# ibm-granite/dolomite-engine

Measured on NVIDIA H100. Metric: tokens_per_sec, higher is better.
Workload: dtype bf16

## Files before the change

dolomite_engine_b200/csrc/attention_fwd.cu:

```cuda
#include "attention_common.cuh"
#include "../../include/dolomite_b200.h"

using namespace dolo;

namespace {

constexpr int FWD_THREADS = 256;
constexpr int KV_STAGES = 2;

struct FwdParams {
    __nv_bfloat16* out;
    float* lse;
    const int32_t* cu_seqlens;
    int n_docs;
    int64_t T;
    int n_groups, q_per_group;
    int n_heads;
    float scale_log2;
    float scale;
    AttnDropout drop;
    int head_chunk;
    int n_tile_slots;
};

template <int HD>
__global__ void __launch_bounds__(FWD_THREADS, 1)
    attn_fwd_kernel(const __grid_constant__ CUtensorMap tmap64, const __grid_constant__ CUtensorMap tmapR,
                    const FwdParams p) {
    using CH = HeadChunks<HD>;
    constexpr int TILE_BYTES = CH::tile_bytes(ATT_TILE);

    int ti, head;
    attn_cta_order(p.head_chunk, p.n_tile_slots, ti, head);
    ti = p.n_tile_slots - 1 - ti;
    const TileLoc loc = locate_tile(p.cu_seqlens, p.n_docs, ti);
    if (!loc.valid) return;
    const int group = head / p.q_per_group, slot = head % p.q_per_group;
    const int q_col = (group * (p.q_per_group + 2) + slot) * HD;
    const int k_col = (group * (p.q_per_group + 2) + p.q_per_group) * HD;
    const int v_col = k_col + HD;
    const int q0 = loc.tile * ATT_TILE;
    const int n_kv = loc.tile + 1;

    extern __shared__ uint8_t smem_raw[];
    uint8_t* smem = smem_align_1024(smem_raw);
    uint8_t* sQ = smem;
    uint8_t* sK = sQ + TILE_BYTES;
    uint8_t* sV = sK + KV_STAGES * TILE_BYTES;
    uint64_t* bars = reinterpret_cast<uint64_t*>(sV + KV_STAGES * TILE_BYTES);
    uint64_t* q_full = bars;
    uint64_t* kv_full = bars + 1;
    uint64_t* kv_empty = bars + 3;

    const int wg = threadIdx.x >> 7, warp = threadIdx.x >> 5, lane = threadIdx.x & 31;

    auto load_kv = [&](int j, int s) {
        mbar_expect_tx(&kv_full[s], 2 * TILE_BYTES);
        tma_load_chunked<HD, ATT_TILE>(sK + s * TILE_BYTES, &tmap64, &tmapR, &kv_full[s], k_col, loc.doc_start + j * ATT_TILE);
        tma_load_chunked<HD, ATT_TILE>(sV + s * TILE_BYTES, &tmap64, &tmapR, &kv_full[s], v_col, loc.doc_start + j * ATT_TILE);
    };
    if (threadIdx.x == 0) {
        if (CH::NC64 > 0) tma_prefetch_desc(&tmap64);
        if (CH::REM > 0) tma_prefetch_desc(&tmapR);
        mbar_init(q_full, 1);
        for (int i = 0; i < KV_STAGES; ++i) {
            mbar_init(&kv_full[i], 1);
            mbar_init(&kv_empty[i], FWD_THREADS / 32);
        }
        mbar_fence_init();
        mbar_expect_tx(q_full, TILE_BYTES);
        tma_load_chunked<HD, ATT_TILE>(sQ, &tmap64, &tmapR, q_full, q_col, loc.doc_start + q0);
        for (int j = 0; j < KV_STAGES && j < n_kv; ++j) load_kv(j, j);
    }
    __syncthreads();

    const int wr = (warp & 3) * 16 + (lane >> 2);
    const int wc = 2 * (lane & 3);
    const int qr[2] = {q0 + wg * 64 + wr, q0 + wg * 64 + wr + 8};
    const bool drop = p.drop.threshold != 0;
    const uint32_t head_key = dropout_head_key(uint32_t(head), p.drop.key0, p.drop.key1);
    const uint32_t sq = smem_u32(sQ);

    float o[HD / 2];
#pragma unroll
    for (int i = 0; i < HD / 2; ++i) o[i] = 0.f;
    float m_run[2] = {-INFINITY, -INFINITY}, l_run[2] = {0.f, 0.f};

    mbar_wait(q_full, 0, 10);
    for (int j = 0; j < n_kv; ++j) {
        const int s = j & (KV_STAGES - 1);
        mbar_wait(&kv_full[s], (j / KV_STAGES) & 1, 11);
        const uint32_t sk = smem_u32(sK + s * TILE_BYTES), sv = smem_u32(sV + s * TILE_BYTES);
        float sc[ATT_TILE / 2];
        wgmma_fence();
#pragma unroll
        for (int c = 0; c < CH::NCHUNK; ++c) {
            const int w = CH::width(c);
#pragma unroll
            for (int k = 0; k < w / 16; ++k)
                wgmma_ss<ATT_TILE, 0, 0>(sc, chunk_desc_kmajor(sq + CH::offset(c, ATT_TILE) + wg * 64 * 2 * w, w, k),
                                         chunk_desc_kmajor(sk + CH::offset(c, ATT_TILE), w, k), (c != 0 || k != 0) ? 1u : 0u);
        }
        wgmma_commit();
        wgmma_wait<0>();
        reg_fence<ATT_TILE / 2>(sc);

        const bool diag = j == loc.tile;
        const int kbase = j * ATT_TILE + wc;
#pragma unroll
        for (int h = 0; h < 2; ++h) {
            float mx = m_run[h];
#pragma unroll
            for (int b = 0; b < ATT_TILE / 8; ++b)
#pragma unroll
                for (int e = 0; e < 2; ++e) {
                    float& x = sc[4 * b + 2 * h + e];
                    if (diag && kbase + 8 * b + e > qr[h]) x = -INFINITY;
                    mx = fmaxf(mx, x);
                }
            mx = fmaxf(mx, __shfl_xor_sync(0xffffffffu, mx, 1));
            mx = fmaxf(mx, __shfl_xor_sync(0xffffffffu, mx, 2));
            const float corr = fast_exp2((m_run[h] - mx) * p.scale_log2);
            const float neg_m = -mx * p.scale_log2;
            float lsum = 0.f;
#pragma unroll
            for (int b = 0; b < ATT_TILE / 8; ++b)
#pragma unroll
                for (int e = 0; e < 2; ++e) {
                    float& x = sc[4 * b + 2 * h + e];
                    float pr = fast_exp2(fmaf(x, p.scale_log2, neg_m));
                    lsum += pr;
                    if (drop)
                        pr *= attn_drop_scale(p.drop, head_key, loc.doc_start + qr[h], loc.doc_start + kbase + 8 * b + e);
                    x = pr;
                }
            l_run[h] = l_run[h] * corr + lsum;
            m_run[h] = mx;
#pragma unroll
            for (int b = 0; b < HD / 8; ++b) {
                o[4 * b + 2 * h] *= corr;
                o[4 * b + 2 * h + 1] *= corr;
            }
        }
        uint32_t pa[ATT_TILE / 16][4];
#pragma unroll
        for (int kk = 0; kk < ATT_TILE / 16; ++kk) acc_to_a_frag(sc, kk, pa[kk]);

        wgmma_fence();
#pragma unroll
        for (int c = 0; c < CH::NCHUNK; ++c) {
#pragma unroll
            for (int kk = 0; kk < ATT_TILE / 16; ++kk) {
                if (CH::width(c) == 64)
                    wgmma_rs<64, 1>(o + CH::col(c) / 2, pa[kk], chunk_desc_mnmajor(sv + CH::offset(c, ATT_TILE), 64, kk), 1u);
                else
                    wgmma_rs<(CH::REM ? CH::REM : 16), 1>(o + CH::col(c) / 2, pa[kk],
                                                          chunk_desc_mnmajor(sv + CH::offset(c, ATT_TILE), CH::REM, kk), 1u);
            }
        }
        wgmma_commit();
        wgmma_wait<0>();
        reg_fence<HD / 2>(o);
        if (lane == 0) mbar_arrive(&kv_empty[s]);
        if (threadIdx.x == 0 && j + KV_STAGES < n_kv) {
            mbar_wait(&kv_empty[s], (j / KV_STAGES) & 1, 12);
            load_kv(j + KV_STAGES, s);
        }
        __syncwarp();
    }

#pragma unroll
    for (int h = 0; h < 2; ++h) {
        float l = l_run[h];
        l += __shfl_xor_sync(0xffffffffu, l, 1);
        l += __shfl_xor_sync(0xffffffffu, l, 2);
        if (qr[h] >= loc.doc_len) continue;
        const float inv_l = l > 0.f ? 1.f / l : 0.f;
        const int64_t row = loc.doc_start + qr[h];
        __nv_bfloat16* orow = p.out + row * (int64_t(p.n_heads) * HD) + int64_t(head) * HD + wc;
#pragma unroll
        for (int b = 0; b < HD / 8; ++b)
            *reinterpret_cast<uint32_t*>(orow + 8 * b) = pack_bf16(o[4 * b + 2 * h] * inv_l, o[4 * b + 2 * h + 1] * inv_l);
        if ((lane & 3) == 0) p.lse[int64_t(head) * p.T + row] = m_run[h] * p.scale + logf(l);
    }
}

template <int HD>
int launch_fwd(const void* qkv, int64_t row_stride, const FwdParams& p, cudaStream_t st) {
    using CH = HeadChunks<HD>;
    CUtensorMap t64, tR;
    int rc = attn_make_maps<HD>(qkv, row_stride, p.T, &t64, &tR);
    if (rc) return rc;
    constexpr int smem_bytes = 1024 + (1 + 2 * KV_STAGES) * CH::tile_bytes(ATT_TILE) + 128;
    static_assert(smem_bytes <= 232448, "attention forward shared memory budget exceeded");
    auto kern = attn_fwd_kernel<HD>;
    static bool attr_set = false;
    if (!attr_set) {
        DOLO_CUDA_OK(cudaFuncSetAttribute(kern, cudaFuncAttributeMaxDynamicSharedMemorySize, smem_bytes));
        attr_set = true;
    }
    const int64_t max_tiles = (p.T + ATT_TILE - 1) / ATT_TILE + p.n_docs;
    DOLO_REQUIRE(max_tiles == p.n_tile_slots && max_tiles * p.n_heads < (1ll << 31), "attn_fwd: grid too large");
    dim3 grid((unsigned)(max_tiles * p.n_heads));
    kern<<<grid, FWD_THREADS, smem_bytes, st>>>(t64, tR, p);
    DOLO_LAUNCH_OK("attn_varlen_fwd");
    return DOLO_OK;
}

}

uint32_t dolo_dropout_threshold(float p);

extern "C" int dolomite_b200_attn_varlen_fwd(const void* qkv, int64_t row_stride, void* out, float* lse,
                                             const int32_t* cu_seqlens, int n_docs, int64_t T, int max_seqlen,
                                             int n_groups, int q_per_group, int head_dim, float softmax_scale,
                                             void* stream) {
    return dolomite_b200_attn_varlen_fwd_dropout(qkv, row_stride, out, lse, cu_seqlens, n_docs, T, max_seqlen, n_groups,
                                                 q_per_group, head_dim, softmax_scale, 0.f, 0, 0, stream);
}

extern "C" int dolomite_b200_attn_varlen_fwd_dropout(const void* qkv, int64_t row_stride, void* out, float* lse,
                                                     const int32_t* cu_seqlens, int n_docs, int64_t T, int max_seqlen,
                                                     int n_groups, int q_per_group, int head_dim, float softmax_scale,
                                                     float dropout_p, uint32_t key0, uint32_t key1, void* stream) {
    DOLO_REQUIRE(dropout_p >= 0.f && dropout_p < 1.f, "attn_fwd: dropout_p=%f must be in [0, 1)", double(dropout_p));
    DOLO_REQUIRE(n_docs >= 0 && T >= 0, "attn_fwd: negative sizes");
// ... 36 lines not shown
```

dolomite_engine_b200/csrc/common.cuh:

```cuda
#pragma once

#include <cuda.h>
#include <cuda_bf16.h>
#include <cuda_runtime.h>
#include <stdint.h>
#include <stdio.h>

extern "C" const char* dolomite_b200_last_error();
int dolo_set_error(const char* fmt, ...);
int dolo_check_cuda(cudaError_t e, const char* what);

#define DOLO_CUDA_OK(expr)                                             \
    do {                                                               \
        cudaError_t _e = (expr);                                       \
        if (_e != cudaSuccess) return dolo_check_cuda(_e, #expr);      \
    } while (0)

#define DOLO_REQUIRE(cond, ...)                                        \
    do {                                                               \
        if (!(cond)) return dolo_set_error(__VA_ARGS__);               \
    } while (0)

#define DOLO_LAUNCH_OK(name)                                           \
    do {                                                               \
// ... 52 lines not shown
    uint32_t ok;
    asm volatile(
        "{\n\t"
        ".reg .pred p;\n\t"
        "mbarrier.try_wait.parity.shared::cta.b64 p, [%1], %2;\n\t"
        "selp.u32 %0, 1, 0, p;\n\t"
        "}\n"
        : "=r"(ok)
        : "r"(smem_u32(bar)), "r"(parity)
        : "memory");
    return ok != 0;
}

#ifndef DOLO_WATCHDOG_CYCLES
#define DOLO_WATCHDOG_CYCLES (8000000000LL)
#endif
__device__ __forceinline__ void mbar_wait(uint64_t* bar, uint32_t parity, int tag = 0) {
    (void)tag;
    if (mbar_try_wait(bar, parity)) return;
    long long t0 = clock64();
    while (!mbar_try_wait(bar, parity)) {
        if (clock64() - t0 > DOLO_WATCHDOG_CYCLES) __trap();
    }
}

__device__ __forceinline__ void fence_proxy_async_smem() {
    asm volatile("fence.proxy.async.shared::cta;" ::: "memory");
}

__device__ __forceinline__ void named_bar_sync(uint32_t id, uint32_t nthreads) {
    asm volatile("bar.sync %0, %1;" ::"r"(id), "r"(nthreads) : "memory");
}

__device__ __forceinline__ void tma_prefetch_desc(const CUtensorMap* m) {
    asm volatile("prefetch.tensormap [%0];" ::"l"(reinterpret_cast<uint64_t>(m)) : "memory");
}
__device__ __forceinline__ void tma_load_2d(void* smem_dst, const CUtensorMap* m, uint64_t* bar, int c0, int c1) {
    asm volatile(
        "cp.async.bulk.tensor.2d.shared::cluster.global.mbarrier::complete_tx::bytes [%0], [%1, {%3, %4}], [%2];"
        ::"r"(smem_u32(smem_dst)), "l"(reinterpret_cast<uint64_t>(m)), "r"(smem_u32(bar)), "r"(c0), "r"(c1)
        : "memory");
}
constexpr uint64_t TMA_HINT_NORMAL = 0x1000000000000000ull;
constexpr uint64_t TMA_HINT_EVICT_FIRST = 0x12F0000000000000ull;
constexpr uint64_t TMA_HINT_EVICT_LAST = 0x14F0000000000000ull;
__device__ __forceinline__ void tma_load_2d_hint(void* smem_dst, const CUtensorMap* m, uint64_t* bar, int c0, int c1,
                                                 uint64_t hint) {
    asm volatile(
        "cp.async.bulk.tensor.2d.shared::cluster.global.mbarrier::complete_tx::bytes.L2::cache_hint [%0], [%1, {%3, %4}], [%2], %5;"
        ::"r"(smem_u32(smem_dst)), "l"(reinterpret_cast<uint64_t>(m)), "r"(smem_u32(bar)), "r"(c0), "r"(c1), "l"(hint)
        : "memory");
}
__device__ __forceinline__ void tma_load_3d(void* smem_dst, const CUtensorMap* m, uint64_t* bar, int c0, int c1,
                                            int c2) {
    asm volatile(
        "cp.async.bulk.tensor.3d.shared::cluster.global.mbarrier::complete_tx::bytes [%0], [%1, {%3, %4, %5}], [%2];"
        ::"r"(smem_u32(smem_dst)), "l"(reinterpret_cast<uint64_t>(m)), "r"(smem_u32(bar)), "r"(c0), "r"(c1), "r"(c2)
        : "memory");
}
__device__ __forceinline__ void tma_store_2d(const CUtensorMap* m, const void* smem_src, int c0, int c1) {
    asm volatile("cp.async.bulk.tensor.2d.global.shared::cta.bulk_group [%0, {%2, %3}], [%1];" ::"l"(
                     reinterpret_cast<uint64_t>(m)),
                 "r"(smem_u32(smem_src)), "r"(c0), "r"(c1)
                 : "memory");
}
__device__ __forceinline__ void tma_reduce_add_2d(const CUtensorMap* m, const void* smem_src, int c0, int c1) {
// ... 37 lines not shown
}
__device__ __forceinline__ void cluster_sync_all() {
    asm volatile("barrier.cluster.arrive.release.aligned;" ::: "memory");
    asm volatile("barrier.cluster.wait.acquire.aligned;" ::: "memory");
}

__device__ __forceinline__ uint64_t gmma_desc(uint32_t saddr, uint32_t lbo_bytes, uint32_t sbo_bytes, uint32_t layout_type) {
    uint64_t d = 0;
    d |= uint64_t((saddr & 0x3FFFFu) >> 4);
    d |= uint64_t((lbo_bytes >> 4) & 0x3FFFu) << 16;
    d |= uint64_t((sbo_bytes >> 4) & 0x3FFFu) << 32;
    d |= uint64_t(layout_type & 3u) << 62;
    return d;
}
__device__ __forceinline__ void wgmma_fence() { asm volatile("wgmma.fence.sync.aligned;" ::: "memory"); }
__device__ __forceinline__ void wgmma_commit() { asm volatile("wgmma.commit_group.sync.aligned;" ::: "memory"); }
template <int N>
__device__ __forceinline__ void wgmma_wait() {
    asm volatile("wgmma.wait_group.sync.aligned %0;" ::"n"(N) : "memory");
}
template <int N>
__device__ __forceinline__ void setmaxnreg_dec() {
    asm volatile("setmaxnreg.dec.sync.aligned.u32 %0;" ::"n"(N));
}
template <int N>
__device__ __forceinline__ void setmaxnreg_inc() {
    asm volatile("setmaxnreg.inc.sync.aligned.u32 %0;" ::"n"(N));
}
template <int N>
__device__ __forceinline__ void reg_fence(float* d) {
#pragma unroll
    for (int i = 0; i < N; ++i) asm volatile("" : "+f"(d[i])::"memory");
}


__device__ __forceinline__ uint32_t pack_bf16(float lo, float hi) {
    __nv_bfloat162 v = __floats2bfloat162_rn(lo, hi);
    return *reinterpret_cast<uint32_t*>(&v);
}
__device__ __forceinline__ float bf16_lo(uint32_t v) { return __uint_as_float(v << 16); }
__device__ __forceinline__ float bf16_hi(uint32_t v) { return __uint_as_float(v & 0xFFFF0000u); }
__device__ __forceinline__ float bf16_round(float x) { return __bfloat162float(__float2bfloat16_rn(x)); }
__device__ __forceinline__ void acc_to_a_frag(const float* d, int kk, uint32_t (&a)[4]) {
    a[0] = pack_bf16(d[8 * kk + 0], d[8 * kk + 1]);
    a[1] = pack_bf16(d[8 * kk + 2], d[8 * kk + 3]);
    a[2] = pack_bf16(d[8 * kk + 4], d[8 * kk + 5]);
    a[3] = pack_bf16(d[8 * kk + 6], d[8 * kk + 7]);
}

__device__ __forceinline__ uint32_t lowbias32(uint32_t x) {
    x ^= x >> 16;
    x *= 0x21f0aaadu;
    x ^= x >> 15;
    x *= 0x735a2d97u;
    x ^= x >> 15;
    return x;
}
__device__ __forceinline__ uint32_t dropout_hash_flat(uint64_t e, uint32_t key0, uint32_t key1) {
    return lowbias32(lowbias32(uint32_t(e) ^ key0) + uint32_t(e >> 32) + key1);
}
__device__ __forceinline__ uint32_t dropout_head_key(uint32_t head, uint32_t key0, uint32_t key1) {
    return lowbias32(head * 0xC2B2AE3Du + key0) ^ key1;
}
__device__ __forceinline__ uint32_t dropout_hash_qk(uint32_t q, uint32_t k, uint32_t head_key) {
    return lowbias32((q * 0x9E3779B1u) ^ (k * 0x85EBCA77u) ^ head_key);
}
// ... 21 lines not shown
```

dolomite_engine_b200/csrc/gemm.cu:

```cuda
#include <string.h>

#include "common.cuh"
#include "wgmma.cuh"
#include "../../include/dolomite_b200.h"

using namespace dolo;

namespace {

constexpr int BM = 128;
constexpr int BN = 128;
constexpr int BK = 64;
constexpr int STAGES = 6;
constexpr int A_STAGE_BYTES = BM * BK * 2;
constexpr int B_STAGE_BYTES = BN * BK * 2;
constexpr int STAGE_BYTES = A_STAGE_BYTES + B_STAGE_BYTES;
constexpr int GEMM_THREADS = 384;
constexpr int SMEM_BYTES = 1024  + STAGES * STAGE_BYTES + 256 ;
static_assert(SMEM_BYTES <= 232448, "shared memory budget exceeded (227 KB per block on sm_90)");

template <int TN>
struct Ring {
    static_assert(TN == 128 || TN == 256, "tile width 128 or 256");
    static constexpr int STAGES = TN == 256 ? 4 : 6;
    static constexpr int B_BYTES = TN * BK * 2;
    static constexpr int STAGE_BYTES = A_STAGE_BYTES + B_BYTES;
    static constexpr int SMEM_BYTES = 1024  + STAGES * STAGE_BYTES + 256 ;
    static_assert(SMEM_BYTES <= 232448, "shared memory budget exceeded (227 KB per block on sm_90)");
};

constexpr int PRODUCER_REGS = 40;
constexpr int CONSUMER_REGS = 232;
static_assert(PRODUCER_REGS * 128 + 2 * CONSUMER_REGS * 128 <= 65536, "register file exceeded");

constexpr double TILE256_COST = 1.81;

constexpr int MAXP = 4;

struct GemmMaps {
    CUtensorMap a[MAXP], b[MAXP];
};

struct Problem {
    void* D;
    const void* C;
    const __nv_bfloat16* bias;
    int64_t ldd, ldc;
    int M, N;
    int num_m, num_n, num_kb;
    int group_m;
    int tile_start;
    float alpha, beta;
    uint64_t hint_a, hint_b;
};

struct GemmParams {
    Problem pr[MAXP];
    int n_prob;
    int num_tiles;
    int d_is_f32;
    int grouped;
    const int* m_tile_group;
    const int* a_row_index;
    const void* gather_a;
    int64_t gather_lda;
    int gather_k;
    int b_group_rows;
    const int* group_k_offsets;
    int num_groups;
    int64_t d_group_stride;
};

struct TileInfo {
    int q;
    int m_blk, n_blk, grp, kb0, kb1;
    bool valid;
};

__device__ __forceinline__ void tile_coords(int t, int num_m, int num_n, int gm, int& m_blk, int& n_blk) {
    const int per_group = gm * num_n;
    const int group = t / per_group;
    const int first_m = group * gm;
    const int gsize = min(num_m - first_m, gm);
    const int r = t - group * per_group;
    m_blk = first_m + r % gsize;
    n_blk = r / gsize;
}

__device__ __forceinline__ TileInfo tile_info(int t, const GemmParams& p) {
    TileInfo ti;
    ti.q = 0;
#pragma unroll
    for (int i = 1; i < MAXP; ++i)
        if (i < p.n_prob && t >= p.pr[i].tile_start) ti.q = i;
    const Problem& pr = p.pr[ti.q];
    t -= pr.tile_start;
    ti.grp = 0;
    ti.kb0 = 0;
    ti.kb1 = pr.num_kb;
    ti.valid = true;
    if (p.grouped == 3) {
        const int per = pr.num_m * pr.num_n;
        const int split = t / per;
        tile_coords(t - split * per, pr.num_m, pr.num_n, pr.group_m, ti.m_blk, ti.n_blk);
        const int kb_per = (pr.num_kb + p.num_groups - 1) / p.num_groups;
        ti.kb0 = split * kb_per;
        ti.kb1 = min(pr.num_kb, ti.kb0 + kb_per);
        ti.valid = ti.kb1 > ti.kb0;
    } else if (p.grouped == 2) {
        const int per = pr.num_m * pr.num_n;
        ti.grp = t / per;
        tile_coords(t - ti.grp * per, pr.num_m, pr.num_n, pr.group_m, ti.m_blk, ti.n_blk);
        ti.kb0 = p.group_k_offsets[ti.grp] / BK;
        ti.kb1 = p.group_k_offsets[ti.grp + 1] / BK;
        ti.valid = ti.kb1 > ti.kb0;
    } else {
        tile_coords(t, pr.num_m, pr.num_n, pr.group_m, ti.m_blk, ti.n_blk);
        if (p.grouped == 1) {
            ti.grp = p.m_tile_group[ti.m_blk];
            ti.valid = ti.grp >= 0;
        }
    }
    return ti;
}

template <bool A_MN, bool B_MN, int TN>
__global__ void __launch_bounds__(GEMM_THREADS, 1)
    gemm_bf16_kernel(const __grid_constant__ GemmMaps maps, const __grid_constant__ GemmParams p) {
    constexpr int STAGES = Ring<TN>::STAGES;
    constexpr int B_STAGE_BYTES = Ring<TN>::B_BYTES;
    constexpr int STAGE_BYTES = Ring<TN>::STAGE_BYTES;
    extern __shared__ uint8_t smem_raw[];
    uint8_t* smem = smem_align_1024(smem_raw);
    uint8_t* smem_a = smem;
    uint8_t* smem_b = smem + STAGES * A_STAGE_BYTES;
    uint64_t* bars = reinterpret_cast<uint64_t*>(smem + STAGES * STAGE_BYTES);
    uint64_t* full_bar = bars;
    uint64_t* empty_bar = bars + STAGES;

    const int wg = threadIdx.x >> 7;
    const int warp = threadIdx.x >> 5;
    const int lane = threadIdx.x & 31;
    const int num_tiles = p.num_tiles;
    const bool gather = TN == 128 && !A_MN && p.a_row_index != nullptr;

    if (threadIdx.x == 0) {
        for (int q = 0; q < p.n_prob; ++q) {
            if (!gather) tma_prefetch_desc(&maps.a[q]);
            tma_prefetch_desc(&maps.b[q]);
        }
        for (int i = 0; i < STAGES; ++i) {
            mbar_init(&full_bar[i], gather ? 33 : 1);
            mbar_init(&empty_bar[i], 8);
        }
        mbar_fence_init();
    }
    __syncthreads();

    if (wg == 0) {
        if constexpr (TN == 256) setmaxnreg_dec<PRODUCER_REGS>();
        if (warp != 0) return;
        if (gather) {
            const __nv_bfloat16* A = static_cast<const __nv_bfloat16*>(p.gather_a);
            int stage = 0;
            uint32_t phase = 0;
            for (int t = blockIdx.x; t < num_tiles; t += gridDim.x) {
                const TileInfo ti = tile_info(t, p);
                if (!ti.valid) continue;
                const CUtensorMap* tmap_b = &maps.b[ti.q];
                const int b_outer = ti.grp * p.b_group_rows;
                const int4 src = *reinterpret_cast<const int4*>(p.a_row_index + int64_t(ti.m_blk) * BM + lane * 4);
                const int srow[4] = {src.x, src.y, src.z, src.w};
                for (int kb = ti.kb0; kb < ti.kb1; ++kb) {
                    mbar_wait(&empty_bar[stage], phase ^ 1, 1);
                    uint8_t* sa = smem_a + stage * A_STAGE_BYTES;
                    uint8_t* sb = smem_b + stage * B_STAGE_BYTES;
                    if (lane == 0) {
                        mbar_expect_tx(&full_bar[stage], B_STAGE_BYTES);
                        if (!B_MN) {
                            tma_load_2d(sb, tmap_b, &full_bar[stage], kb * BK, b_outer + ti.n_blk * BN);
                        } else {
#pragma unroll
                            for (int i = 0; i < BN / 64; ++i)
                                tma_load_2d(sb + i * (BK * 128), tmap_b, &full_bar[stage], ti.n_blk * BN + i * 64,
                                            b_outer + kb * BK);
                        }
                    }
// ... 23 lines not shown
                const CUtensorMap* tmap_b = &maps.b[ti.q];
                const uint64_t ha = p.pr[ti.q].hint_a, hb = p.pr[ti.q].hint_b;
                const int m_blk = ti.m_blk, n_blk = ti.n_blk;
                const int b_outer = (p.grouped == 1) ? ti.grp * p.b_group_rows : 0;
                for (int kb = ti.kb0; kb < ti.kb1; ++kb) {
                    mbar_wait(&empty_bar[stage], phase ^ 1, 1);
                    uint8_t* sa = smem_a + stage * A_STAGE_BYTES;
                    uint8_t* sb = smem_b + stage * B_STAGE_BYTES;
                    mbar_expect_tx(&full_bar[stage], STAGE_BYTES);
                    if (!A_MN) {
                        tma_load_2d_hint(sa, tmap_a, &full_bar[stage], kb * BK, m_blk * BM, ha);
                    } else {
#pragma unroll
                        for (int i = 0; i < BM / 64; ++i)
                            tma_load_2d_hint(sa + i * (BK * 128), tmap_a, &full_bar[stage], m_blk * BM + i * 64, kb * BK, ha);
                    }
                    if (!B_MN) {
                        tma_load_2d_hint(sb, tmap_b, &full_bar[stage], kb * BK, b_outer + n_blk * TN, hb);
                    } else {
#pragma unroll
                        for (int i = 0; i < TN / 64; ++i)
                            tma_load_2d_hint(sb + i * (BK * 128), tmap_b, &full_bar[stage], n_blk * TN + i * 64,
                                             b_outer + kb * BK, hb);
                    }
                    if (++stage == STAGES) { stage = 0; phase ^= 1; }
                }
            }
        }
        return;
    }

    if constexpr (TN == 256) setmaxnreg_inc<CONSUMER_REGS>();
    const int cw = wg - 1;
    const int wr = (warp & 3) * 16 + (lane >> 2);
    const int wc = 2 * (lane & 3);
    int stage = 0;
    uint32_t phase = 0;
    float acc[TN / 2];
    for (int t = blockIdx.x; t < num_tiles; t += gridDim.x) {
        const TileInfo ti = tile_info(t, p);
        const Problem& pr = p.pr[ti.q];
        const int64_t row0 = int64_t(ti.m_blk) * BM + cw * 64 + wr;
        const int col0 = ti.n_blk * TN + wc;
        if (!ti.valid) {
            if (p.grouped == 2 && p.d_is_f32 && pr.C == nullptr) {
                float* D = static_cast<float*>(pr.D) + int64_t(ti.grp) * p.d_group_stride;
#pragma unroll
                for (int h = 0; h < 2; ++h) {
                    const int64_t row = row0 + 8 * h;
                    if (row >= pr.M) continue;
                    for (int j = 0; j < TN / 8; ++j)
                        if (col0 + 8 * j < pr.N)
                            *reinterpret_cast<float2*>(D + row * pr.ldd + col0 + 8 * j) = make_float2(0.f, 0.f);
                }
            }
            continue;
        }
        int prev_stage = -1;
        for (int kb = ti.kb0; kb < ti.kb1; ++kb) {
            mbar_wait(&full_bar[stage], phase, 3);
            wgmma_fence();
            const uint32_t sa = smem_u32(smem_a + stage * A_STAGE_BYTES);
            const uint32_t sb = smem_u32(smem_b + stage * B_STAGE_BYTES);
#pragma unroll
            for (int k = 0; k < BK / 16; ++k) {
                const uint64_t adesc = A_MN ? gmma_desc(sa + cw * (BK * 128) + k * 2048, BK * 128, 1024, 1)
                                            : gmma_desc(sa + cw * (64 * 128) + k * 32, 16, 1024, 1);
                const uint64_t bdesc = B_MN ? gmma_desc(sb + k * 2048, BK * 128, 1024, 1) : gmma_desc(sb + k * 32, 16, 1024, 1);
                wgmma_ss<TN, A_MN ? 1 : 0, B_MN ? 1 : 0>(acc, adesc, bdesc, (kb != ti.kb0 || k != 0) ? 1u : 0u);
            }
            wgmma_commit();
            wgmma_wait<1>();
            if (prev_stage >= 0 && lane == 0) mbar_arrive(&empty_bar[prev_stage]);
            prev_stage = stage;
            if (++stage == STAGES) { stage = 0; phase ^= 1; }
        }
        wgmma_wait<0>();
        reg_fence<TN / 2>(acc);
        if (prev_stage >= 0 && lane == 0) mbar_arrive(&empty_bar[prev_stage]);

        const int64_t d_off = (p.grouped == 2) ? int64_t(ti.grp) * p.d_group_stride : 0;
        const float alpha = pr.alpha, beta = pr.beta;
        const __nv_bfloat16* bias = pr.bias;
        const int N = pr.N;
#pragma unroll
        for (int j = 0; j < TN / 8; ++j) {
            const int col = col0 + 8 * j;
            if (col >= N) continue;
            float b0 = 0.f, b1 = 0.f;
            if (bias != nullptr) {
                const uint32_t bv = *reinterpret_cast<const uint32_t*>(bias + col);
                b0 = bf16_lo(bv);
                b1 = bf16_hi(bv);
            }
#pragma unroll
            for (int h = 0; h < 2; ++h) {
                const int64_t row = row0 + 8 * h;
                if (row >= pr.M) continue;
                float v0 = (acc[4 * j + 2 * h] + b0) * alpha;
                float v1 = (acc[4 * j + 2 * h + 1] + b1) * alpha;
                if (p.d_is_f32) {
                    float* d = static_cast<float*>(pr.D) + d_off + row * pr.ldd + col;
                    if (p.grouped == 3) {
                        asm volatile("red.global.add.v2.f32 [%0], {%1, %2};" ::"l"(d), "f"(v0), "f"(v1) : "memory");
                        continue;
                    }
                    if (pr.C) {
                        const float2 c2 = *reinterpret_cast<const float2*>(static_cast<const float*>(pr.C) + d_off + row * pr.ldc + col);
                        v0 += beta * c2.x;
                        v1 += beta * c2.y;
                    }
                    *reinterpret_cast<float2*>(d) = make_float2(v0, v1);
                } else {
                    __nv_bfloat16* d = static_cast<__nv_bfloat16*>(pr.D) + d_off + row * pr.ldd + col;
                    if (pr.C) {
                        const uint32_t cv =
                            *reinterpret_cast<const uint32_t*>(static_cast<const __nv_bfloat16*>(pr.C) + d_off + row * pr.ldc + col);
                        v0 += beta * bf16_lo(cv);
                        v1 += beta * bf16_hi(cv);
                    }
                    *reinterpret_cast<uint32_t*>(d) = pack_bf16(v0, v1);
                }
            }
        }
    }
}

int gemm_workers() {
    const int sms = dolo_num_sms() - dolo_option_gemm_sm_margin();
    return sms < 1 ? 1 : sms;
}

template <bool A_MN, bool B_MN, int TN>
int launch_gemm(const GemmMaps& maps, const GemmParams& p, cudaStream_t st) {
    auto kern = gemm_bf16_kernel<A_MN, B_MN, TN>;
    constexpr int smem_bytes = Ring<TN>::SMEM_BYTES;
    static bool attr_set = false;
    if (!attr_set) {
        DOLO_CUDA_OK(cudaFuncSetAttribute(kern, cudaFuncAttributeMaxDynamicSharedMemorySize, smem_bytes));
        attr_set = true;
    }
    const int sms = gemm_workers();
    const int grid = p.num_tiles < sms ? p.num_tiles : sms;
    kern<<<grid, GEMM_THREADS, smem_bytes, st>>>(maps, p);
    DOLO_LAUNCH_OK("gemm_bf16");
    return DOLO_OK;
}

int choose_tile_n(int n, const int64_t* M, const int64_t* N) {
    const int forced = dolo_option_gemm_tile_n();
    if (forced != 0) return forced;
    const int64_t w = gemm_workers();
    int64_t t128 = 0, t256 = 0;
    for (int q = 0; q < n; ++q) {
        const int64_t mb = (M[q] + BM - 1) / BM;
        t128 += mb * ((N[q] + 127) / 128);
        t256 += mb * ((N[q] + 255) / 256);
    }
// ... 215 lines not shown
    DOLO_REQUIRE(!a_mn_major || M % 8 == 0, "gemm: MN-major A requires M %% 8 == 0");
    DOLO_REQUIRE(g.C == nullptr || g.ldc % (d_is_f32 ? 4 : 8) == 0, "gemm: ldc alignment");
    DOLO_REQUIRE(M < (1ll << 31) && N < (1ll << 31) && K < (1ll << 31), "gemm: dimension too large");
    uint64_t dims[2], strides[2];
    uint32_t box[2];
    int rc;
    if (ga.a_row_index != nullptr) {
        DOLO_REQUIRE(!a_mn_major, "gemm: gather-on-load needs a K-major A");
        DOLO_REQUIRE((reinterpret_cast<uintptr_t>(g.A) & 15) == 0, "gemm: gather-on-load needs a 16-byte aligned A");
        p.gather_a = g.A;
        p.gather_lda = g.lda;
        p.gather_k = int(K);
    } else {
        if (!a_mn_major) {
            dims[0] = uint64_t(K); dims[1] = uint64_t(M); strides[0] = 2; strides[1] = uint64_t(g.lda) * 2;
            box[0] = BK; box[1] = BM;
        } else {
            dims[0] = uint64_t(M); dims[1] = uint64_t(K); strides[0] = 2; strides[1] = uint64_t(g.lda) * 2;
            box[0] = 64; box[1] = BK;
        }
        rc = dolo_make_tmap(&maps.a[q], g.A, 2, 2, dims, strides, box, DOLO_SW_128);
        if (rc) return rc;
    }
    strides[0] = 2;
    if (!b_mn_major) {
        dims[0] = uint64_t(K); dims[1] = uint64_t(ga.mode == 1 ? ga.b_total_outer : N); strides[1] = uint64_t(g.ldb) * 2;
        box[0] = BK; box[1] = uint32_t(tile_n);
    } else {
        dims[0] = uint64_t(N); dims[1] = uint64_t(ga.mode == 1 ? ga.b_total_outer : K); strides[1] = uint64_t(g.ldb) * 2;
        box[0] = 64; box[1] = BK;
    }
    rc = dolo_make_tmap(&maps.b[q], g.B, 2, 2, dims, strides, box, DOLO_SW_128);
    if (rc) return rc;
    Problem& pr = p.pr[q];
    pr.D = g.D;
    pr.C = g.C;
    pr.bias = static_cast<const __nv_bfloat16*>(g.bias);
    pr.ldd = g.ldd;
    pr.ldc = g.ldc;
    pr.M = int(M);
    pr.N = int(N);
    pr.alpha = g.alpha;
    pr.beta = g.C ? g.beta : 0.f;
    pr.hint_a = pr.hint_b = TMA_HINT_NORMAL;
    if (dolo_option_gemm_l2_hints() && ga.mode == 0 && K >= 4096 && (M + N) * K * 2 > (24ll << 20)) {
        const bool a_smaller = M <= N;
        pr.hint_a = a_smaller ? TMA_HINT_EVICT_LAST : TMA_HINT_EVICT_FIRST;
        pr.hint_b = a_smaller ? TMA_HINT_EVICT_FIRST : TMA_HINT_EVICT_LAST;
    }
    pr.num_m = int((M + BM - 1) / BM);
    pr.num_n = int((N + tile_n - 1) / tile_n);
    pr.num_kb = int((K + BK - 1) / BK);
    {
        const int64_t panel_bytes = int64_t(BM) * K * 2;
        int64_t gm = (12ll << 20) / (panel_bytes > 0 ? panel_bytes : 1);
        if (gm < 4) gm = 4;
        if (gm > 64) gm = 64;
        pr.group_m = int(gm);
    }
    return DOLO_OK;
}

template <int TN>
static int dispatch_layout(int a_mn_major, int b_mn_major, const GemmMaps& maps, const GemmParams& p, cudaStream_t st) {
    if (!a_mn_major && !b_mn_major) return launch_gemm<false, false, TN>(maps, p, st);
    if (!a_mn_major && b_mn_major) return launch_gemm<false, true, TN>(maps, p, st);
    if (a_mn_major && !b_mn_major) return launch_gemm<true, false, TN>(maps, p, st);
    return launch_gemm<true, true, TN>(maps, p, st);
}

static int dispatch(int tile_n, int a_mn_major, int b_mn_major, const GemmMaps& maps, const GemmParams& p, cudaStream_t st) {
    return tile_n == 256 ? dispatch_layout<256>(a_mn_major, b_mn_major, maps, p, st)
                         : dispatch_layout<128>(a_mn_major, b_mn_major, maps, p, st);
}

static int gemm_impl(const void* A, int64_t lda, int a_mn_major, const void* B, int64_t ldb, int b_mn_major, void* D,
                     int64_t ldd, int d_is_f32, const void* C, int64_t ldc, float alpha, float beta, const void* bias,
                     int64_t M, int64_t N, int64_t K, int flags, void* stream, const GroupArgs& ga) {
    DOLO_REQUIRE(M >= 0 && N >= 0 && K >= 0, "gemm: negative dimension");
    if (M == 0 || N == 0) return DOLO_OK;
    const bool tma_store = (flags & DOLO_GEMM_FLAG_TMA_STORE) != 0;
    DOLO_REQUIRE(!tma_store || (!d_is_f32 && C == nullptr), "gemm: TMA-store epilogue needs bf16 D and no C");
    const int tile_n = ga.mode == 0 ? choose_tile_n(1, &M, &N) : BN;
    GemmMaps maps;
    GemmParams p;
    memset(&p, 0, sizeof(p));
    GemmProblemArgs g{A, lda, B, ldb, D, ldd, C, ldc, bias, alpha, beta, M, N, K};
    int rc = setup_problem(maps, p, 0, g, a_mn_major, b_mn_major, d_is_f32, ga, tile_n);
    if (rc) return rc;
    p.n_prob = 1;
    p.pr[0].tile_start = 0;
    p.num_tiles = p.pr[0].num_m * p.pr[0].num_n * (ga.mode >= 2 ? ga.num_groups : 1);
    p.d_is_f32 = d_is_f32;
    p.grouped = ga.mode;
    p.m_tile_group = ga.m_tile_group;
    p.a_row_index = ga.a_row_index;
    p.b_group_rows = int(ga.b_group_rows);
    p.group_k_offsets = ga.group_k_offsets;
    p.num_groups = ga.num_groups;
    p.d_group_stride = ga.d_group_stride;
    return dispatch(tile_n, a_mn_major, b_mn_major, maps, p, static_cast<cudaStream_t>(stream));
}

extern "C" int dolomite_b200_gemm_bf16_wgrad_multi(int n_problems, const void* const* dY, const int64_t* ld_dy,
                                                   const void* const* X, const int64_t* ld_x, float* const* dW,
                                                   const int64_t* ld_dw, const int64_t* M, const int64_t* N, int64_t K,
                                                   const float* alpha, const int* accumulate, void* stream) {
    DOLO_REQUIRE(n_problems >= 1 && n_problems <= MAXP, "wgrad_multi: between 1 and %d problems per launch", MAXP);
    for (int q = 0; q < n_problems; ++q) DOLO_REQUIRE(M[q] > 0 && N[q] > 0, "wgrad_multi: empty problem %d", q);
    const int tile_n = choose_tile_n(n_problems, M, N);
    GemmMaps maps;
    GemmParams p;
    memset(&p, 0, sizeof(p));
    int tiles = 0;
    for (int q = 0; q < n_problems; ++q) {
        GemmProblemArgs g{dY[q], ld_dy[q], X[q], ld_x[q], dW[q], ld_dw[q], accumulate[q] ? dW[q] : nullptr, ld_dw[q], nullptr,
                          alpha[q], 1.f, M[q], N[q], K};
        int rc = setup_problem(maps, p, q, g, 1, 1, 1, GroupArgs(), tile_n);
        if (rc) return rc;
        p.pr[q].tile_start = tiles;
        tiles += p.pr[q].num_m * p.pr[q].num_n;
    }
    p.n_prob = n_problems;
    p.num_tiles = tiles;
    p.d_is_f32 = 1;
    p.grouped = 0;
    p.num_groups = 1;
    return dispatch(tile_n, 1, 1, maps, p, static_cast<cudaStream_t>(stream));
}

extern "C" int dolomite_b200_gemm_bf16_tile_n(int n_problems, const int64_t* M, const int64_t* N, int* tile_n,
                                              float* cost_256_over_128) {
    DOLO_REQUIRE(n_problems >= 1 && n_problems <= MAXP && M != nullptr && N != nullptr && tile_n != nullptr,
// ... 185 lines not shown
```

Before: 12030.

## Overlap softmax with next QK^T wgmma and deepen KV pipeline stages

Restructures the attention forward loop so that the S=QK^T wgmma for tile j+1 and the PV wgmma for tile j are in flight together, and the softmax of j+1 runs while PV completes. This hides tensor-core latency behind exponent math. The KV ring buffer also grows from 2 to 4 stages when shared memory allows, with the barrier offsets and the release logic adjusted for it. The cost is higher register pressure from the extra live S/P fragments, and a KV slot is now refilled one iteration later.

```diff
diff --git a/dolomite_engine_b200/csrc/attention_fwd.cu b/dolomite_engine_b200/csrc/attention_fwd.cu
--- a/dolomite_engine_b200/csrc/attention_fwd.cu
+++ b/dolomite_engine_b200/csrc/attention_fwd.cu
@@ -6,7 +6,10 @@
 namespace {
 
 constexpr int FWD_THREADS = 256;
-constexpr int KV_STAGES = 2;
+template <int HD>
+constexpr int fwd_kv_stages() {
+    return (1 + 2 * 4) * HeadChunks<HD>::tile_bytes(ATT_TILE) + 1024 + 128 <= 232448 ? 4 : 3;
+}
 
 struct FwdParams {
     __nv_bfloat16* out;
@@ -29,6 +32,7 @@
                     const FwdParams p) {
     using CH = HeadChunks<HD>;
     constexpr int TILE_BYTES = CH::tile_bytes(ATT_TILE);
+    constexpr int KV_STAGES = fwd_kv_stages<HD>();
 
     int ti, head;
     attn_cta_order(p.head_chunk, p.n_tile_slots, ti, head);
@@ -50,7 +54,7 @@
     uint64_t* bars = reinterpret_cast<uint64_t*>(sV + KV_STAGES * TILE_BYTES);
     uint64_t* q_full = bars;
     uint64_t* kv_full = bars + 1;
-    uint64_t* kv_empty = bars + 3;
+    uint64_t* kv_empty = kv_full + KV_STAGES;
 
     const int wg = threadIdx.x >> 7, warp = threadIdx.x >> 5, lane = threadIdx.x & 31;
 
@@ -85,13 +89,14 @@
 #pragma unroll
     for (int i = 0; i < HD / 2; ++i) o[i] = 0.f;
     float m_run[2] = {-INFINITY, -INFINITY}, l_run[2] = {0.f, 0.f};
-
-    mbar_wait(q_full, 0, 10);
-    for (int j = 0; j < n_kv; ++j) {
-        const int s = j & (KV_STAGES - 1);
+    float sc[ATT_TILE / 2];
+    uint32_t pa[ATT_TILE / 16][4];
+    float corr[2];
+
+    auto issue_s = [&](int j) {
+        const int s = j % KV_STAGES;
         mbar_wait(&kv_full[s], (j / KV_STAGES) & 1, 11);
-        const uint32_t sk = smem_u32(sK + s * TILE_BYTES), sv = smem_u32(sV + s * TILE_BYTES);
-        float sc[ATT_TILE / 2];
+        const uint32_t sk = smem_u32(sK + s * TILE_BYTES);
         wgmma_fence();
 #pragma unroll
         for (int c = 0; c < CH::NCHUNK; ++c) {
@@ -102,9 +107,24 @@
                                          chunk_desc_kmajor(sk + CH::offset(c, ATT_TILE), w, k), (c != 0 || k != 0) ? 1u : 0u);
         }
         wgmma_commit();
-        wgmma_wait<0>();
-        reg_fence<ATT_TILE / 2>(sc);
-
+    };
+    auto issue_pv = [&](int j) {
+        const uint32_t sv = smem_u32(sV + (j % KV_STAGES) * TILE_BYTES);
+        wgmma_fence();
+#pragma unroll
+        for (int c = 0; c < CH::NCHUNK; ++c) {
+#pragma unroll
+            for (int kk = 0; kk < ATT_TILE / 16; ++kk) {
+                if (CH::width(c) == 64)
+                    wgmma_rs<64, 1>(o + CH::col(c) / 2, pa[kk], chunk_desc_mnmajor(sv + CH::offset(c, ATT_TILE), 64, kk), 1u);
+                else
+                    wgmma_rs<(CH::REM ? CH::REM : 16), 1>(o + CH::col(c) / 2, pa[kk],
+                                                          chunk_desc_mnmajor(sv + CH::offset(c, ATT_TILE), CH::REM, kk), 1u);
+            }
+        }
+        wgmma_commit();
+    };
+    auto softmax = [&](int j) {
         const bool diag = j == loc.tile;
         const int kbase = j * ATT_TILE + wc;
 #pragma unroll
@@ -120,7 +140,7 @@
                 }
             mx = fmaxf(mx, __shfl_xor_sync(0xffffffffu, mx, 1));
             mx = fmaxf(mx, __shfl_xor_sync(0xffffffffu, mx, 2));
-            const float corr = fast_exp2((m_run[h] - mx) * p.scale_log2);
+            corr[h] = fast_exp2((m_run[h] - mx) * p.scale_log2);
             const float neg_m = -mx * p.scale_log2;
             float lsum = 0.f;
 #pragma unroll
@@ -134,40 +154,55 @@
                         pr *= attn_drop_scale(p.drop, head_key, loc.doc_start + qr[h], loc.doc_start + kbase + 8 * b + e);
                     x = pr;
                 }
-            l_run[h] = l_run[h] * corr + lsum;
+            l_run[h] = l_run[h] * corr[h] + lsum;
             m_run[h] = mx;
+        }
+    };
+    auto rescale_and_pack = [&]() {
+#pragma unroll
+        for (int h = 0; h < 2; ++h)
 #pragma unroll
             for (int b = 0; b < HD / 8; ++b) {
-                o[4 * b + 2 * h] *= corr;
-                o[4 * b + 2 * h + 1] *= corr;
+                o[4 * b + 2 * h] *= corr[h];
+                o[4 * b + 2 * h + 1] *= corr[h];
             }
-        }
-        uint32_t pa[ATT_TILE / 16][4];
 #pragma unroll
         for (int kk = 0; kk < ATT_TILE / 16; ++kk) acc_to_a_frag(sc, kk, pa[kk]);
-
-        wgmma_fence();
-#pragma unroll
-        for (int c = 0; c < CH::NCHUNK; ++c) {
-#pragma unroll
-            for (int kk = 0; kk < ATT_TILE / 16; ++kk) {
-                if (CH::width(c) == 64)
-                    wgmma_rs<64, 1>(o + CH::col(c) / 2, pa[kk], chunk_desc_mnmajor(sv + CH::offset(c, ATT_TILE), 64, kk), 1u);
-                else
-                    wgmma_rs<(CH::REM ? CH::REM : 16), 1>(o + CH::col(c) / 2, pa[kk],
-                                                          chunk_desc_mnmajor(sv + CH::offset(c, ATT_TILE), CH::REM, kk), 1u);
-            }
-        }
-        wgmma_commit();
+        reg_fence<HD / 2>(o);
+        reg_fence_u32<ATT_TILE / 4>(&pa[0][0]);
+    };
+    auto release = [&](int j) {
+        if (lane == 0) mbar_arrive(&kv_empty[j % KV_STAGES]);
+        const int m = j - 1;
+        if (threadIdx.x == 0 && m >= 0 && m + KV_STAGES < n_kv) {
+            const int sm = m % KV_STAGES;
+            mbar_wait(&kv_empty[sm], (m / KV_STAGES) & 1, 12);
+            load_kv(m + KV_STAGES, sm);
+        }
+        __syncwarp();
+    };
+
+    mbar_wait(q_full, 0, 10);
+    issue_s(0);
+    wgmma_wait<0>();
+    reg_fence<ATT_TILE / 2>(sc);
+    softmax(0);
+    rescale_and_pack();
+    for (int j = 0; j + 1 < n_kv; ++j) {
+        issue_s(j + 1);
+        issue_pv(j);
+        wgmma_wait<1>();
+        reg_fence<ATT_TILE / 2>(sc);
+        softmax(j + 1);
         wgmma_wait<0>();
         reg_fence<HD / 2>(o);
-        if (lane == 0) mbar_arrive(&kv_empty[s]);
-        if (threadIdx.x == 0 && j + KV_STAGES < n_kv) {
-            mbar_wait(&kv_empty[s], (j / KV_STAGES) & 1, 12);
-            load_kv(j + KV_STAGES, s);
-        }
-        __syncwarp();
-    }
+        release(j);
+        rescale_and_pack();
+    }
+    issue_pv(n_kv - 1);
+    wgmma_wait<0>();
+    reg_fence<HD / 2>(o);
+    release(n_kv - 1);
 
 #pragma unroll
     for (int h = 0; h < 2; ++h) {
@@ -191,7 +226,7 @@
     CUtensorMap t64, tR;
     int rc = attn_make_maps<HD>(qkv, row_stride, p.T, &t64, &tR);
     if (rc) return rc;
-    constexpr int smem_bytes = 1024 + (1 + 2 * KV_STAGES) * CH::tile_bytes(ATT_TILE) + 128;
+    constexpr int smem_bytes = 1024 + (1 + 2 * fwd_kv_stages<HD>()) * CH::tile_bytes(ATT_TILE) + 128;
     static_assert(smem_bytes <= 232448, "attention forward shared memory budget exceeded");
     auto kern = attn_fwd_kernel<HD>;
     static bool attr_set = false;
diff --git a/dolomite_engine_b200/csrc/common.cuh b/dolomite_engine_b200/csrc/common.cuh
--- a/dolomite_engine_b200/csrc/common.cuh
+++ b/dolomite_engine_b200/csrc/common.cuh
@@ -211,6 +211,11 @@
 #pragma unroll
     for (int i = 0; i < N; ++i) asm volatile("" : "+f"(d[i])::"memory");
 }
+template <int N>
+__device__ __forceinline__ void reg_fence_u32(uint32_t* a) {
+#pragma unroll
+    for (int i = 0; i < N; ++i) asm volatile("" : "+r"(a[i])::"memory");
+}
 
 
 __device__ __forceinline__ uint32_t pack_bf16(float lo, float hi) {
```

Measured after the change: 12010, median of 6. About the same (-0.2%).

## Route GEMM epilogue through swizzled smem slabs with TMA store and C prefetch

Applied to the files above, without the earlier changes.

Replaces the direct per-thread global stores in the GEMM epilogue with a double-buffered shared-memory slab path. Results go through stmatrix or float2 writes into 128B-swizzled slabs and are written out by TMA store or reduce-add, and the C operand is prefetched by TMA during the mainloop. Bias is staged in shared memory, and the tile-256 cost heuristic is lowered so wider tiles are picked more often. The aim is fully coalesced async output writes that overlap the next tile's mainloop, at the cost of extra smem, named-barrier syncs and more complexity in the boundary handling done by the tensor maps.

```diff
diff --git a/dolomite_engine_b200/csrc/common.cuh b/dolomite_engine_b200/csrc/common.cuh
--- a/dolomite_engine_b200/csrc/common.cuh
+++ b/dolomite_engine_b200/csrc/common.cuh
@@ -108,6 +108,18 @@
     asm volatile("bar.sync %0, %1;" ::"r"(id), "r"(nthreads) : "memory");
 }
 
+__device__ __forceinline__ void stmatrix_x4(uint32_t saddr, const uint32_t (&r)[4]) {
+    asm volatile("stmatrix.sync.aligned.m8n8.x4.shared.b16 [%0], {%1, %2, %3, %4};" ::"r"(saddr), "r"(r[0]), "r"(r[1]),
+                 "r"(r[2]), "r"(r[3])
+                 : "memory");
+}
+__device__ __forceinline__ void ldmatrix_x4(uint32_t saddr, uint32_t (&r)[4]) {
+    asm volatile("ldmatrix.sync.aligned.m8n8.x4.shared.b16 {%0, %1, %2, %3}, [%4];"
+                 : "=r"(r[0]), "=r"(r[1]), "=r"(r[2]), "=r"(r[3])
+                 : "r"(saddr)
+                 : "memory");
+}
+
 __device__ __forceinline__ void tma_prefetch_desc(const CUtensorMap* m) {
     asm volatile("prefetch.tensormap [%0];" ::"l"(reinterpret_cast<uint64_t>(m)) : "memory");
 }
diff --git a/dolomite_engine_b200/csrc/gemm.cu b/dolomite_engine_b200/csrc/gemm.cu
--- a/dolomite_engine_b200/csrc/gemm.cu
+++ b/dolomite_engine_b200/csrc/gemm.cu
@@ -19,13 +19,22 @@
 constexpr int SMEM_BYTES = 1024  + STAGES * STAGE_BYTES + 256 ;
 static_assert(SMEM_BYTES <= 232448, "shared memory budget exceeded (227 KB per block on sm_90)");
 
+constexpr int EPI_SLAB_BYTES = 64 * 128;
+constexpr int EPI_BYTES = 2  * 2  * EPI_SLAB_BYTES;
+constexpr int EPI_BIAS_BYTES = 2  * 256 * 2;
+
 template <int TN>
 struct Ring {
     static_assert(TN == 128 || TN == 256, "tile width 128 or 256");
     static constexpr int STAGES = TN == 256 ? 4 : 6;
     static constexpr int B_BYTES = TN * BK * 2;
     static constexpr int STAGE_BYTES = A_STAGE_BYTES + B_BYTES;
-    static constexpr int SMEM_BYTES = 1024  + STAGES * STAGE_BYTES + 256 ;
+    static constexpr int EPI_OFFSET = STAGES * STAGE_BYTES;
+    static constexpr int BIAS_OFFSET = EPI_OFFSET + EPI_BYTES;
+    static constexpr int BAR_OFFSET = BIAS_OFFSET + EPI_BIAS_BYTES;
+    static constexpr int SMEM_BYTES = 1024  + BAR_OFFSET + 256 ;
+    static_assert(EPI_OFFSET % 1024 == 0, "epilogue slabs must stay 1024-byte aligned");
+    static_assert((2 * STAGES + 4) * 8 <= 256, "barrier area");
     static_assert(SMEM_BYTES <= 232448, "shared memory budget exceeded (227 KB per block on sm_90)");
 };
 
@@ -33,12 +42,12 @@
 constexpr int CONSUMER_REGS = 232;
 static_assert(PRODUCER_REGS * 128 + 2 * CONSUMER_REGS * 128 <= 65536, "register file exceeded");
 
-constexpr double TILE256_COST = 1.81;
+constexpr double TILE256_COST = 1.65;
 
 constexpr int MAXP = 4;
 
 struct GemmMaps {
-    CUtensorMap a[MAXP], b[MAXP];
+    CUtensorMap a[MAXP], b[MAXP], d[MAXP], c[MAXP];
 };
 
 struct Problem {
@@ -68,7 +77,6 @@
     int b_group_rows;
     const int* group_k_offsets;
     int num_groups;
-    int64_t d_group_stride;
 };
 
 struct TileInfo {
@@ -124,6 +132,142 @@
     return ti;
 }
 
+struct Epilogue {
+    uint8_t* slabs;
+    uint32_t* bias;
+    uint64_t* c_bar;
+    int slab = 0;
+    uint32_t c_phase = 0;
+    int cw;
+    bool leader;
+
+    __device__ __forceinline__ void load_c_prefetch(const CUtensorMap* cmap, int chunk_cols, int col0, int row0, int grp) {
+        tma_store_wait_read<0>();
+#pragma unroll
+        for (int i = 0; i < 2; ++i) {
+            const int s = slab ^ i;
+            mbar_expect_tx(&c_bar[s], EPI_SLAB_BYTES);
+            tma_load_3d(slabs + s * EPI_SLAB_BYTES, cmap, &c_bar[s], col0 + i * chunk_cols, row0, grp);
+        }
+    }
+
+    __device__ __forceinline__ void begin_tile() {
+        if (leader) tma_store_wait_read<0>();
+        named_bar_sync(1 + cw, 128);
+    }
+
+    __device__ __forceinline__ void reuse_slab(bool has_c, const CUtensorMap* cmap, int col, int row0, int grp) {
+        if (leader) {
+            tma_store_wait_read<1>();
+            if (has_c) {
+                mbar_expect_tx(&c_bar[slab], EPI_SLAB_BYTES);
+                tma_load_3d(slabs + slab * EPI_SLAB_BYTES, cmap, &c_bar[slab], col, row0, grp);
+            }
+        }
+        named_bar_sync(1 + cw, 128);
+    }
+
+    template <int TN, bool F32>
+    __device__ __forceinline__ void store(const float (&acc)[TN / 2], const CUtensorMap* dmap, const CUtensorMap* cmap,
+                                          int col0, int row0, int grp, float alpha, float beta, bool has_bias, bool has_c,
+                                          bool reduce) {
+        constexpr int CHUNK = F32 ? 32 : 64;
+        constexpr int NB = CHUNK / 8;
+        const int lane = threadIdx.x & 31;
+        const int wrow = ((threadIdx.x >> 5) & 3) * 16;
+#pragma unroll
+        for (int ch = 0; ch < TN / CHUNK; ++ch) {
+            uint8_t* sl = slabs + slab * EPI_SLAB_BYTES;
+            if (ch >= 2) reuse_slab(has_c, cmap, col0 + ch * CHUNK, row0, grp);
+            if (has_c) {
+                mbar_wait(&c_bar[slab], (c_phase >> slab) & 1u, 4);
+                c_phase ^= 1u << slab;
+            }
+            if constexpr (F32) {
+#pragma unroll
+                for (int jj = 0; jj < NB; ++jj) {
+                    const int j = ch * NB + jj;
+                    float b0 = 0.f, b1 = 0.f;
+                    if (has_bias) {
+                        const uint32_t bv = bias[4 * j + (lane & 3)];
+                        b0 = bf16_lo(bv);
+                        b1 = bf16_hi(bv);
+                    }
+#pragma unroll
+                    for (int h = 0; h < 2; ++h) {
+                        const int r = wrow + 8 * h + (lane >> 2);
+                        const int byte = jj * 32 + (lane & 3) * 8;
+                        float2* s = reinterpret_cast<float2*>(sl + r * 128 + ((((byte >> 4) ^ (r & 7)) << 4) | (byte & 15)));
+                        float v0 = (acc[4 * j + 2 * h] + b0) * alpha;
+                        float v1 = (acc[4 * j + 2 * h + 1] + b1) * alpha;
+                        if (has_c) {
+                            const float2 c2 = *s;
+                            v0 += beta * c2.x;
+                            v1 += beta * c2.y;
+                        }
+                        *s = make_float2(v0, v1);
+                    }
+                }
+            } else {
+                const int m = lane >> 3;
+                const int r = wrow + 8 * (m & 1) + (lane & 7);
+#pragma unroll
+                for (int jj = 0; jj < NB; jj += 2) {
+                    const uint32_t addr = smem_u32(sl + r * 128 + (((jj + (m >> 1)) ^ (lane & 7)) << 4));
+                    uint32_t cv[4], out[4];
+                    if (has_c) ldmatrix_x4(addr, cv);
+#pragma unroll
+                    for (int i = 0; i < 4; ++i) {
+                        const int j = ch * NB + jj + (i >> 1), h = i & 1;
+                        float b0 = 0.f, b1 = 0.f;
+                        if (has_bias) {
+                            const uint32_t bv = bias[4 * j + (lane & 3)];
+                            b0 = bf16_lo(bv);
+                            b1 = bf16_hi(bv);
+                        }
+                        float v0 = (acc[4 * j + 2 * h] + b0) * alpha;
+                        float v1 = (acc[4 * j + 2 * h + 1] + b1) * alpha;
+                        if (has_c) {
+                            v0 += beta * bf16_lo(cv[i]);
+                            v1 += beta * bf16_hi(cv[i]);
+                        }
+                        out[i] = pack_bf16(v0, v1);
+                    }
+                    stmatrix_x4(addr, out);
+                }
+            }
+            issue(dmap, col0 + ch * CHUNK, row0, grp, reduce);
+        }
+    }
+
+    template <int TN>
+    __device__ __forceinline__ void store_zero_f32(const CUtensorMap* dmap, int col0, int row0, int grp) {
+        begin_tile();
+#pragma unroll 1
+        for (int ch = 0; ch < TN / 32; ++ch) {
+            if (ch >= 2) reuse_slab(false, nullptr, 0, 0, 0);
+            uint4* s = reinterpret_cast<uint4*>(slabs + slab * EPI_SLAB_BYTES);
+#pragma unroll
+            for (int i = 0; i < EPI_SLAB_BYTES / 16 / 128; ++i) s[(threadIdx.x & 127) + 128 * i] = make_uint4(0u, 0u, 0u, 0u);
+            issue(dmap, col0 + ch * 32, row0, grp, false);
+        }
+    }
+
+    __device__ __forceinline__ void issue(const CUtensorMap* dmap, int col, int row0, int grp, bool reduce) {
+        const uint8_t* sl = slabs + slab * EPI_SLAB_BYTES;
+        fence_proxy_async_smem();
+        named_bar_sync(1 + cw, 128);
+        if (leader) {
+            if (reduce)
+                tma_reduce_add_3d(dmap, sl, col, row0, grp);
+            else
+                tma_store_3d(dmap, sl, col, row0, grp);
+            tma_store_commit();
+        }
+        slab ^= 1;
+    }
+};
+
 template <bool A_MN, bool B_MN, int TN>
 __global__ void __launch_bounds__(GEMM_THREADS, 1)
     gemm_bf16_kernel(const __grid_constant__ GemmMaps maps, const __grid_constant__ GemmParams p) {
@@ -134,9 +278,10 @@
     uint8_t* smem = smem_align_1024(smem_raw);
     uint8_t* smem_a = smem;
     uint8_t* smem_b = smem + STAGES * A_STAGE_BYTES;
-    uint64_t* bars = reinterpret_cast<uint64_t*>(smem + STAGES * STAGE_BYTES);
+    uint64_t* bars = reinterpret_cast<uint64_t*>(smem + Ring<TN>::BAR_OFFSET);
     uint64_t* full_bar = bars;
     uint64_t* empty_bar = bars + STAGES;
+    uint64_t* c_bar = bars + 2 * STAGES;
 
     const int wg = threadIdx.x >> 7;
     const int warp = threadIdx.x >> 5;
@@ -153,6 +298,7 @@
             mbar_init(&full_bar[i], gather ? 33 : 1);
             mbar_init(&empty_bar[i], 8);
         }
+        for (int i = 0; i < 4; ++i) mbar_init(&c_bar[i], 1);
         mbar_fence_init();
     }
     __syncthreads();
@@ -242,30 +388,32 @@
 
     if constexpr (TN == 256) setmaxnreg_inc<CONSUMER_REGS>();
     const int cw = wg - 1;
-    const int wr = (warp & 3) * 16 + (lane >> 2);
-    const int wc = 2 * (lane & 3);
+    const int wt = threadIdx.x & 127;
+    Epilogue epi;
+    epi.slabs = smem + Ring<TN>::EPI_OFFSET + cw * 2 * EPI_SLAB_BYTES;
+    epi.bias = reinterpret_cast<uint32_t*>(smem + Ring<TN>::BIAS_OFFSET + cw * (EPI_BIAS_BYTES / 2));
+    epi.c_bar = c_bar + 2 * cw;
+    epi.cw = cw;
+    epi.leader = wt == 0;
+    const int chunk_cols = p.d_is_f32 ? 32 : 64;
     int stage = 0;
     uint32_t phase = 0;
     float acc[TN / 2];
     for (int t = blockIdx.x; t < num_tiles; t += gridDim.x) {
         const TileInfo ti = tile_info(t, p);
         const Problem& pr = p.pr[ti.q];
-        const int64_t row0 = int64_t(ti.m_blk) * BM + cw * 64 + wr;
-        const int col0 = ti.n_blk * TN + wc;
+        const int row0 = ti.m_blk * BM + cw * 64;
+        const int col0 = ti.n_blk * TN;
+        const int dgrp = p.grouped == 2 ? ti.grp : 0;
         if (!ti.valid) {
-            if (p.grouped == 2 && p.d_is_f32 && pr.C == nullptr) {
-                float* D = static_cast<float*>(pr.D) + int64_t(ti.grp) * p.d_group_stride;
-#pragma unroll
-                for (int h = 0; h < 2; ++h) {
-                    const int64_t row = row0 + 8 * h;
-                    if (row >= pr.M) continue;
-                    for (int j = 0; j < TN / 8; ++j)
-                        if (col0 + 8 * j < pr.N)
-                            *reinterpret_cast<float2*>(D + row * pr.ldd + col0 + 8 * j) = make_float2(0.f, 0.f);
-                }
-            }
+            if (p.grouped == 2 && p.d_is_f32 && pr.C == nullptr) epi.store_zero_f32<TN>(&maps.d[ti.q], col0, row0, dgrp);
             continue;
         }
+        const bool has_bias = pr.bias != nullptr;
+        const bool has_c = pr.C != nullptr;
+        uint32_t bias_v = 0;
+        if (has_bias && wt < TN / 2 && col0 + 2 * wt < pr.N)
+            bias_v = __ldg(reinterpret_cast<const uint32_t*>(pr.bias + col0 + 2 * wt));
         int prev_stage = -1;
         for (int kb = ti.kb0; kb < ti.kb1; ++kb) {
             mbar_wait(&full_bar[stage], phase, 3);
@@ -276,10 +424,12 @@
             for (int k = 0; k < BK / 16; ++k) {
                 const uint64_t adesc = A_MN ? gmma_desc(sa + cw * (BK * 128) + k * 2048, BK * 128, 1024, 1)
                                             : gmma_desc(sa + cw * (64 * 128) + k * 32, 16, 1024, 1);
-                const uint64_t bdesc = B_MN ? gmma_desc(sb + k * 2048, BK * 128, 1024, 1) : gmma_desc(sb + k * 32, 16, 1024, 1);
+                const uint64_t bdesc = B_MN ? gmma_desc(sb + k * 2048, BK * 128, 1024, 1)
+                                            : gmma_desc(sb + k * 32, 16, 1024, 1);
                 wgmma_ss<TN, A_MN ? 1 : 0, B_MN ? 1 : 0>(acc, adesc, bdesc, (kb != ti.kb0 || k != 0) ? 1u : 0u);
             }
             wgmma_commit();
+            if (kb == min(ti.kb0 + 2, ti.kb1 - 1) && has_c && epi.leader) epi.load_c_prefetch(&maps.c[ti.q], chunk_cols, col0, row0, dgrp);
             wgmma_wait<1>();
             if (prev_stage >= 0 && lane == 0) mbar_arrive(&empty_bar[prev_stage]);
             prev_stage = stage;
@@ -288,52 +438,17 @@
         wgmma_wait<0>();
         reg_fence<TN / 2>(acc);
         if (prev_stage >= 0 && lane == 0) mbar_arrive(&empty_bar[prev_stage]);
-
-        const int64_t d_off = (p.grouped == 2) ? int64_t(ti.grp) * p.d_group_stride : 0;
-        const float alpha = pr.alpha, beta = pr.beta;
-        const __nv_bfloat16* bias = pr.bias;
-        const int N = pr.N;
-#pragma unroll
-        for (int j = 0; j < TN / 8; ++j) {
-            const int col = col0 + 8 * j;
-            if (col >= N) continue;
-            float b0 = 0.f, b1 = 0.f;
-            if (bias != nullptr) {
-                const uint32_t bv = *reinterpret_cast<const uint32_t*>(bias + col);
-                b0 = bf16_lo(bv);
-                b1 = bf16_hi(bv);
-            }
-#pragma unroll
-            for (int h = 0; h < 2; ++h) {
-                const int64_t row = row0 + 8 * h;
-                if (row >= pr.M) continue;
-                float v0 = (acc[4 * j + 2 * h] + b0) * alpha;
-                float v1 = (acc[4 * j + 2 * h + 1] + b1) * alpha;
-                if (p.d_is_f32) {
-                    float* d = static_cast<float*>(pr.D) + d_off + row * pr.ldd + col;
-                    if (p.grouped == 3) {
-                        asm volatile("red.global.add.v2.f32 [%0], {%1, %2};" ::"l"(d), "f"(v0), "f"(v1) : "memory");
-                        continue;
-                    }
-                    if (pr.C) {
-                        const float2 c2 = *reinterpret_cast<const float2*>(static_cast<const float*>(pr.C) + d_off + row * pr.ldc + col);
-                        v0 += beta * c2.x;
-                        v1 += beta * c2.y;
-                    }
-                    *reinterpret_cast<float2*>(d) = make_float2(v0, v1);
-                } else {
-                    __nv_bfloat16* d = static_cast<__nv_bfloat16*>(pr.D) + d_off + row * pr.ldd + col;
-                    if (pr.C) {
-                        const uint32_t cv =
-                            *reinterpret_cast<const uint32_t*>(static_cast<const __nv_bfloat16*>(pr.C) + d_off + row * pr.ldc + col);
-                        v0 += beta * bf16_lo(cv);
-                        v1 += beta * bf16_hi(cv);
-                    }
-                    *reinterpret_cast<uint32_t*>(d) = pack_bf16(v0, v1);
-                }
-            }
-        }
-    }
+        if (has_bias && wt < TN / 2) epi.bias[wt] = bias_v;
+        epi.begin_tile();
+
+        if (p.d_is_f32)
+            epi.store<TN, true>(acc, &maps.d[ti.q], &maps.c[ti.q], col0, row0, dgrp, pr.alpha, pr.beta, has_bias, has_c,
+                                p.grouped == 3);
+        else
+            epi.store<TN, false>(acc, &maps.d[ti.q], &maps.c[ti.q], col0, row0, dgrp, pr.alpha, pr.beta, has_bias, has_c,
+                                 false);
+    }
+    if (epi.leader) tma_store_wait_all<0>();
 }
 
 int gemm_workers() {
@@ -615,6 +730,22 @@
     }
     rc = dolo_make_tmap(&maps.b[q], g.B, 2, 2, dims, strides, box, DOLO_SW_128);
     if (rc) return rc;
+    {
+        const uint64_t eb = d_is_f32 ? 4 : 2;
+        const int64_t groups = ga.mode == 2 ? ga.num_groups : 1;
+        const int64_t group_stride = ga.mode == 2 ? ga.d_group_stride : M * g.ldd;
+        uint64_t ddims[3] = {uint64_t(N), uint64_t(M), uint64_t(groups)};
+        uint64_t dstrides[3] = {eb, uint64_t(g.ldd) * eb, uint64_t(group_stride) * eb};
+        const uint32_t dbox[3] = {uint32_t(128 / eb), 64, 1};
+        rc = dolo_make_tmap(&maps.d[q], g.D, int(eb), 3, ddims, dstrides, dbox, DOLO_SW_128);
+        if (rc) return rc;
+        if (g.C != nullptr) {
+            dstrides[1] = uint64_t(g.ldc) * eb;
+            if (ga.mode != 2) dstrides[2] = uint64_t(M * g.ldc) * eb;
+            rc = dolo_make_tmap(&maps.c[q], g.C, int(eb), 3, ddims, dstrides, dbox, DOLO_SW_128);
+            if (rc) return rc;
+        }
+    }
     Problem& pr = p.pr[q];
     pr.D = g.D;
     pr.C = g.C;
@@ -681,7 +812,6 @@
     p.b_group_rows = int(ga.b_group_rows);
     p.group_k_offsets = ga.group_k_offsets;
     p.num_groups = ga.num_groups;
-    p.d_group_stride = ga.d_group_stride;
     return dispatch(tile_n, a_mn_major, b_mn_major, maps, p, static_cast<cudaStream_t>(stream));
 }
 
```

Measured after the change: 15320 before, 16810 after, median of 6. 1.1x the previous value.
